# vision-agh/apse_uav

Hardware: AMD Instinct MI355X
Metric: 4K UAV frames/sec (whole node) (higher is better)
Workload: dtype f32

## Files before the change

apse_uav_amd/csrc/apse_common.h:

```cpp
#pragma once
#include <hip/hip_runtime.h>
#include <stdint.h>

#define APSE_OK 0
#define APSE_E_INVALID (-1)
#define APSE_E_HIP (-2)
#define APSE_E_NOMEM (-3)
#define APSE_E_STATE (-4)
#define APSE_E_MISSING (-5)
#define APSE_MAX_FRAME_W 49152
#define APSE_MAX_FRAME_H 32768
#define APSE_MAX_CLASSES 80
#define APSE_LDS_BYTES 163840

typedef __attribute__((ext_vector_type(16))) float f32x16;
typedef __attribute__((ext_vector_type(4))) float f32x4;

struct ConvParams {
    const float* x;
    const float* w;
    const uint16_t* w16;
    const float* bias;
    const float* res;
    float* y;
    float* ws;
    int* tile_cnt;
    const int* m_count;
    int m_per_item;
    int m_hint;
    int B, H, W, cin_log2;
    int OH, OW, Cout;
    int KH, KW, stride, pad;
    int KWCp;
    int M;
    int relu;
    int res_mode;
    int out_mode;
    int y_ld, y_coff;
    int cdec;
    int splitk;
    int steps_total;
    const void* next_w;
    unsigned next_w_bytes;
    int prec;
    int x_st, res_st, y_st;
    int no_stream;
};

int apse_launch_conv(const ConvParams& p, int cfg, hipStream_t s, hipEvent_t ev0 = nullptr, hipEvent_t ev1 = nullptr);
int apse_conv_pick_cfg(int M, int Cout, int steps, int* splitk);
#define APSE_CFG_STREAM 9
#define APSE_CFG_BNECK 10
#define APSE_CFG_GLDS 11
#define APSE_CFG_STEMPOOL 12
#define APSE_CFG_SKINNY 13
#define APSE_NCFG 14
bool apse_conv1x1_stream_ok(const ConvParams& p);
int apse_launch_conv1x1_stream(const ConvParams& p, hipStream_t s, hipEvent_t ev0 = nullptr, hipEvent_t ev1 = nullptr);
bool apse_conv_glds16_ok(const ConvParams& p);
bool apse_conv_glds16_small(const ConvParams& p);
bool apse_conv_skinny_ok(const ConvParams& p);
int apse_launch_conv_skinny(const ConvParams& p, hipStream_t s, hipEvent_t ev0 = nullptr, hipEvent_t ev1 = nullptr);
int apse_launch_conv_glds16(const ConvParams& p, hipStream_t s, hipEvent_t ev0 = nullptr, hipEvent_t ev1 = nullptr);
int apse_conv_effective_cfg(const ConvParams& p, int cfg);
typedef __bf16 bf16x8 __attribute__((ext_vector_type(8)));

#ifdef __HIPCC__
typedef _Float16 f16x4_t __attribute__((ext_vector_type(4)));
typedef __bf16 bf16x4_t __attribute__((ext_vector_type(4)));
__device__ __forceinline__ f32x4 apse_ld4(const void* base, size_t idx, int st) {
    if (st == 0) return *reinterpret_cast<const f32x4*>(reinterpret_cast<const float*>(base) + idx);
    f32x4 r;
    if (st == 1) {
        const uint2 raw = *reinterpret_cast<const uint2*>(reinterpret_cast<const uint16_t*>(base) + idx);
        r[0] = __uint_as_float(raw.x << 16); r[1] = __uint_as_float(raw.x & 0xffff0000u);
        r[2] = __uint_as_float(raw.y << 16); r[3] = __uint_as_float(raw.y & 0xffff0000u);
    } else {
        const f16x4_t h = *reinterpret_cast<const f16x4_t*>(reinterpret_cast<const uint16_t*>(base) + idx);
        r[0] = (float)h[0]; r[1] = (float)h[1]; r[2] = (float)h[2]; r[3] = (float)h[3];
    }
    return r;
}
#ifndef APSE_NT
#define APSE_NT 1
#endif
#if APSE_NT
#define APSE_NT_STORE(v, ptr) __builtin_nontemporal_store(v, ptr)
#else
#define APSE_NT_STORE(v, ptr) (*(ptr) = (v))
#endif
__device__ __forceinline__ float apse_relu(float x) {
    float r;
    asm("v_max_f32 %0, 0, %1" : "=v"(r) : "v"(x));
    return r;
}
__device__ __forceinline__ void apse_st4(void* base, size_t idx, f32x4 v, int st) {
    if (st == 0) { APSE_NT_STORE(v, reinterpret_cast<f32x4*>(reinterpret_cast<float*>(base) + idx)); return; }
    if (st == 1) {
        bf16x4_t b;
        b[0] = (__bf16)v[0]; b[1] = (__bf16)v[1]; b[2] = (__bf16)v[2]; b[3] = (__bf16)v[3];
        APSE_NT_STORE(b, reinterpret_cast<bf16x4_t*>(reinterpret_cast<uint16_t*>(base) + idx));
    } else {
        f16x4_t h;
        h[0] = (_Float16)v[0]; h[1] = (_Float16)v[1]; h[2] = (_Float16)v[2]; h[3] = (_Float16)v[3];
        APSE_NT_STORE(h, reinterpret_cast<f16x4_t*>(reinterpret_cast<uint16_t*>(base) + idx));
    }
}
struct ApseWarm { f32x4 v[4]; };
__device__ __forceinline__ void apse_warm_issue(ApseWarm& wv, const void* w, unsigned bytes, unsigned blk, unsigned nblk, int tid) {
    const unsigned stride = (bytes / nblk + 1023u) & ~1023u;
    const unsigned len = stride > 16384u ? 16384u : stride;
    const unsigned lo = blk * stride;
#pragma unroll
    for (int i = 0; i < 4; ++i) {
        const unsigned o = (unsigned)(i * 256 + tid) * 16u;
        wv.v[i] = f32x4{0.f, 0.f, 0.f, 0.f};
        if (w && o < len && lo + o + 16u <= bytes) wv.v[i] = *reinterpret_cast<const f32x4*>(reinterpret_cast<const char*>(w) + lo + o);
    }
}
__device__ __forceinline__ void apse_warm_retire(ApseWarm& wv) {
#pragma unroll
    for (int i = 0; i < 4; ++i) asm volatile("" ::"v"(wv.v[i]));
}
typedef float f32x8 __attribute__((ext_vector_type(8)));
typedef _Float16 f16x8_t __attribute__((ext_vector_type(8)));

__device__ __forceinline__ f32x8 apse_cvt8(const uint4 raw, int st) {
    f32x8 r;
    if (st == 1) {
        r[0] = __uint_as_float(raw.x << 16); r[1] = __uint_as_float(raw.x & 0xffff0000u);
        r[2] = __uint_as_float(raw.y << 16); r[3] = __uint_as_float(raw.y & 0xffff0000u);
        r[4] = __uint_as_float(raw.z << 16); r[5] = __uint_as_float(raw.z & 0xffff0000u);
        r[6] = __uint_as_float(raw.w << 16); r[7] = __uint_as_float(raw.w & 0xffff0000u);
    } else {
        f16x8_t h;
        __builtin_memcpy(&h, &raw, 16);
#pragma unroll
        for (int k = 0; k < 8; ++k) r[k] = (float)h[k];
    }
    return r;
}

__device__ __forceinline__ void apse_st8(void* base, size_t idx, const f32x8& v, int st) {
    if (st == 0) {
        apse_st4(base, idx, f32x4{v[0], v[1], v[2], v[3]}, 0);
        apse_st4(base, idx + 4, f32x4{v[4], v[5], v[6], v[7]}, 0);
    } else if (st == 1) {
// ... 22 lines not shown
```

apse_uav_amd/csrc/detector.hip:

```cpp
#include "apse_common.h"
#include "../../include/apse_hip.h"
#include "preproc_pixel.h"

#include <math.h>
#include <stdio.h>
#include <string.h>

#include <map>
#include <mutex>
#include <string>
#include <vector>

struct RpnLevel { const float* head; int H, W, stride; int n; int k; float base[3][4]; };
struct RpnLevels { RpnLevel lv[5]; int head_ld; int pre_topk; };
struct TopkJob { int kind; int level; int begin, count; int nsrc; int src[4]; int src_count[4]; int dst; int dst_count; };
struct FpnMaps { const void* p[4]; int H[4], W[4]; float scale[4]; int st; };
struct PasteParams {
    const float* boxes; const int* cls; const int* total; const float* logits; int M, ldc; float sx, sy; int out_h, out_w;
    int words_per_row; float thresh; float* boxes_out; int* valid; int* rect; uint64_t* bits; unsigned long long* sums;
};
extern "C" {
int apse_k_pil_resize(const uint8_t*, uint8_t*, void*, int, uint8_t*, const int*, const int*, int, const int*, const int*, int, int,
                      int, int, int, int, int, int, const float*, const UndistortParams*, const LabTables*, const void*, const int*, int, hipStream_t);
int apse_k_undistort_build_map_compact(const UndistortParams*, void*, int*, hipStream_t);
int apse_k_chw_norm(const float*, void*, int, int, int, int, int, int, const float*, hipStream_t);
int apse_k_maxpool3x3s2(const void*, void*, int, int, int, int, int, hipStream_t);
bool apse_assoc_fc_ok(int K, int N);
int apse_k_assoc_fc(const float*, const float*, const float*, float*, const int*, int, int, int, float*, float*, hipStream_t);
int apse_k_stem_pool16(const void*, const uint16_t*, const float*, void*, int, int, int, int, hipStream_t, hipEvent_t, hipEvent_t);
int apse_k_subsample2(const void*, void*, int, int, int, int, int, hipStream_t);
int apse_k_bottleneck64_fused16(const void*, const void*, void*, const uint16_t*, const float*, const uint16_t*, const float*,
                                const uint16_t*, const float*, int, int, int, int, int, hipStream_t, hipEvent_t, hipEvent_t);
int apse_k_nhwc_to_nchw(const void*, float*, int, int, int, int, hipStream_t);
int apse_k_rpn_topk_stage(const RpnLevels*, const TopkJob*, int, uint64_t*, int, int, uint32_t*, hipStream_t);
int apse_k_rpn_decode(const RpnLevels*, int, const uint64_t*, int, const int*, float, float, float, float*, float*, int*,
                      uint32_t*, int, int, hipStream_t);
int apse_k_nms_percat(const float*, const float*, const int*, int, int, int, const uint32_t*, float, int*, int*, int,
                      void*, int, int, int, hipStream_t);
size_t apse_nms_scratch_bytes(int slots);
int apse_k_rank_final(const float*, const float*, int, const int*, const int*, int, int, float*, float*, int*, int*, uint32_t*,
                      int, hipStream_t);
int apse_k_box_candidates(const float*, int, int, const float*, const int*, int, float, float, float, const float*, float,
                          float*, float*, int*, uint32_t*, float*, int, hipStream_t);
int apse_k_box_candidates_wide(const float*, int, int, const float*, const int*, int, float, float, float, const float*, float,
                               float*, float*, int*, uint32_t*, float*, int*, int*, int, hipStream_t);
int apse_k_nms_lists(const float*, const float*, int, const int*, int*, int, const uint32_t*, float, int*, int*, int, void*, int,
                     hipStream_t);
int apse_k_rank_wide(const float*, const float*, int, const int*, const int*, int, int, float*, float*, int*, int*, int, hipStream_t);
int apse_k_pack_detections(const float*, const float*, const int*, const int*, int, int, int, float*, float*, int*, int*,
                           int*, int*, int*, unsigned long long*, hipStream_t);
int apse_k_roi_align(const FpnMaps*, const float*, const int*, const int*, const int*, int, int, int, void*, int, hipStream_t);
int apse_k_roi_pool(const void*, int, int, int, const float*, const int*, const int*, int, int, float, float*, int, int, hipStream_t);
int apse_k_mask_resize(const uint8_t*, int, int, int, int, int, float*, hipStream_t);
int apse_k_round16(const float*, uint16_t*, size_t, int, hipStream_t);
int apse_k_roi_align_masked(const void*, int, int, int, int, const float*, const float*, int, int, int, float, float*, hipStream_t);
int apse_k_l2_normalize(const float*, float*, int, const int*, int, hipStream_t);
int apse_k_sqdist(const float*, const float*, int, int, int, float*, hipStream_t);
int apse_k_mask_paste(const PasteParams*, int, unsigned long long*, int, hipStream_t);
int apse_k_closest_points(const uint64_t*, const int*, const int*, const unsigned long long*, const int*, const int*, const int*, int,
                          int, int, int, int, int*, int*, unsigned long long*, int, hipStream_t);
int apse_k_closest_single(const uint64_t*, int, int, int, float, float, unsigned long long*, hipStream_t);
int apse_k_undistort_gamma(const UndistortParams*, const uint8_t*, uint8_t*, const LabTables*, int, hipStream_t);
int apse_k_bits_to_dense(const uint64_t*, const int*, int, int, int, uint8_t*, hipStream_t);
int apse_k_copy_mask_windows(const uint64_t*, uint64_t*, int, const long long*, const long long*, const int*, const int*, int, hipStream_t);
int apse_k_dense_to_bits(const uint8_t*, int, int, int, uint64_t*, unsigned long long*, hipStream_t);
}

static std::string g_create_error;
#define NMS_SLOT 1024
#define APSE_NARROW_CLASSES 6
#define APSE_EV_HALF 1024
#define APSE_EXPECTED_DETS 8

struct HostW { std::vector<float> v; std::vector<int64_t> shape; };
struct Tens { float* p = nullptr; int H = 0, W = 0, C = 0; int st = 0; };

struct ConvStep {
    ConvParams p;
    int b_mult = 1;
    int fixed_items = 0;
    int cfg = 0;
    double flops_per_item = 0;
    int count_kind = 0;
    void* pool_y = nullptr;
    std::string name;
};
enum StepKind { S_CONV, S_MAXPOOL, S_SUBSAMPLE, S_BNECK };
struct Step { StepKind kind; ConvStep c; const float* x; float* y; int H, W, C; int st = 0; ConvParams p2, p3; };

struct apse_ctx {
    apse_config cfg;
    std::string err;
    std::map<std::string, HostW> hw;
    bool finalized = false;
    int PH = 0, PW = 0;
    std::vector<void*> allocs;
    std::map<std::string, Tens> t;
    std::vector<Step> backbone, rpnhead, boxhead, maskhead, embedfc;
    float* ws = nullptr; size_t ws_floats = 0; int* tile_cnt = nullptr;
    int *hb = nullptr, *hc = nullptr, *vb = nullptr, *vc = nullptr; int hk = 0, vk = 0; uint8_t* rs_tmp = nullptr;
    int rs_pitch = 0;
    int* hcT = nullptr;
    RpnLevels rl_host; RpnLevels* rl_dev = nullptr;
    std::vector<std::vector<TopkJob>> stages; std::vector<TopkJob*> stage_dev; int nslots = 0; uint64_t* lists = nullptr;
    int final_slot_host[5]; int* final_slot_dev = nullptr;
    float *dec_boxes = nullptr, *dec_scores = nullptr; int* dec_valid = nullptr; uint32_t* maxc = nullptr;
    int *keep_idx = nullptr, *keep_cnt = nullptr; void* nms_scratch = nullptr;
    float *props = nullptr, *prop_scores = nullptr; int *prop_entry = nullptr;
    FpnMaps fm;
    float *cand_boxes = nullptr, *cand_scores = nullptr, *probs = nullptr; int* cand_valid = nullptr;
    int pred_ld = 32;
    bool wide = false;
    int *cls_list = nullptr, *cls_cnt = nullptr;
    float *det_boxes = nullptr, *det_scores = nullptr; int *det_entry = nullptr, *det_cnt = nullptr;
    apse_results_layout lay; uint8_t* res = nullptr;
    uint64_t* bits2[2] = {nullptr, nullptr}; int bits_cur = 0, bits_read = 0;
    unsigned long long* sums = nullptr; int wpr = 0; bool sums_dirty = false;
    float* emb_raw = nullptr;
    float* ws_assoc = nullptr;
    float* rf_mask = nullptr; size_t rf_mask_floats = 0;
    bool box_maxc_clean = false;
    UndistortParams cam; bool cam_on = false; LabTables* cam_lut = nullptr; void* cam_map = nullptr; bool cam_map_ok = false;
    int hint_total = 8;
    hipEvent_t read_ev = nullptr; void* read_pending = nullptr;
    uint8_t* given_host[2] = {nullptr, nullptr}; hipEvent_t given_ev[2] = {nullptr, nullptr}; int given_k = 0;
    bool prof_on = false; std::vector<hipEvent_t> ev_pool; int ev_used = 0;
    struct Pending { int cfg; double flops_per_item; int count_kind; int b_mult; int batch; int e0, e1; };
    std::vector<Pending> pending; double prof[APSE_NCFG][3] = {{0}};
    int ev_base = 0, cal_read = -1; std::vector<Pending> pending_read;
    uint64_t* op_bits = nullptr; unsigned long long* op_sums = nullptr; size_t op_bits_words = 0;
};

static int fail(apse_ctx* c, int code, const std::string& msg) {
    if (c) c->err = msg; else g_create_error = msg;
    return code;
}
#define HIPCHK(c, call)                                                                        \
    do {                                                                                       \
        hipError_t e_ = (call);                                                                \
        if (e_ != hipSuccess) return fail(c, APSE_E_HIP, std::string(#call) + ": " + hipGetErrorString(e_)); \
    } while (0)

template <typename T>
static T* dalloc(apse_ctx* c, size_t n, bool zero = true) {
    void* p = nullptr;
    if (hipMalloc(&p, n * sizeof(T) > 0 ? n * sizeof(T) : 16) != hipSuccess) return nullptr;
    if (zero) hipMemset(p, 0, n * sizeof(T));
    c->allocs.push_back(p);
    return reinterpret_cast<T*>(p);
}
template <typename T>
static T* dupload(apse_ctx* c, const std::vector<T>& v) {
    T* p = dalloc<T>(c, v.size(), false);
    if (p && !v.empty()) hipMemcpy(p, v.data(), v.size() * sizeof(T), hipMemcpyHostToDevice);
    return p;
}

static void pack_oihw(const float* w, int Cout, int Cin, int KH, int KW, int cin_p, const float* scale, float* out,
                      int KWCp) {
    for (int o = 0; o < Cout; ++o) {
        const float sc = scale ? scale[o] : 1.0f;
        for (int r = 0; r < KH; ++r)
            for (int s = 0; s < KW; ++s)
                for (int ci = 0; ci < Cin; ++ci)
                    out[((size_t)o * KH + r) * KWCp + s * cin_p + ci] = w[(((size_t)o * Cin + ci) * KH + r) * KW + s] * sc;
    }
}
static int pow2_at_least(int v) { int p = 4; while (p < v) p <<= 1; return p; }

static const HostW* getw(apse_ctx* c, const std::string& n) {
    auto it = c->hw.find(n);
    return it == c->hw.end() ? nullptr : &it->second;
}

static Tens make_t(apse_ctx* c, const std::string& name, int items, int H, int W, int C, int st = 0) {
    Tens t;
    t.H = H; t.W = W; t.C = C; t.st = st;
    const size_t elems = (size_t)items * H * W * C;
    t.p = dalloc<float>(c, st ? (elems + 1) / 2 : elems);
    c->t[name] = t;
    return t;
}

struct ConvSpec {
    std::string name; std::vector<std::string> wnames;
    int KH, KW, stride, pad, relu;
    int fc_h = 0, fc_w = 0;
    int deconv = 0;
    int s2d = 0;
};

static uint16_t round16(float v, int dtype) {
    if (dtype == 2) {
        const _Float16 hval = (_Float16)v;
        uint16_t r;
        memcpy(&r, &hval, 2);
        return r;
    }
    uint32_t b;
    memcpy(&b, &v, 4);
    if ((b & 0x7fffffffu) > 0x7f800000u) return (uint16_t)((b >> 16) | 0x40);
    return (uint16_t)((b + 0x7fffu + ((b >> 16) & 1u)) >> 16);
}
static int storage_type(const apse_ctx* c) { return (c->cfg.compute_dtype >= 1 && c->cfg.storage16) ? c->cfg.compute_dtype : 0; }

static int add_conv(apse_ctx* c, std::vector<Step>& plan, const ConvSpec& sp, const Tens& in, int in_items_mult, Tens* out,
                    const std::string& out_name, const Tens* res, int res_mode, int y_ld_override, int count_kind,
                    float* out_ptr_override = nullptr, const Tens* out_view = nullptr) {
    std::vector<float> rows;
    std::vector<float> bias;
    int Cout = 0, Cin = 0;
    const int KH = sp.KH, KW = sp.KW;
    for (const auto& wn : sp.wnames) {
        const HostW* w = getw(c, wn + ".weight");
        if (!w) return fail(c, APSE_E_MISSING, "missing weight " + wn + ".weight");
        int co, ci;
        std::vector<float> oihw;
        if (sp.fc_h > 0) {
            co = (int)w->shape[0];
            const int flat = (int)w->shape[1];
            ci = flat / (sp.fc_h * sp.fc_w);
            oihw = w->v;
        } else if (sp.deconv) {
            ci = (int)w->shape[0];
            const int cc = (int)w->shape[1];
            co = 4 * cc;
            oihw.assign((size_t)co * ci, 0.f);
            for (int i = 0; i < ci; ++i)
                for (int o = 0; o < cc; ++o)
                    for (int dy = 0; dy < 2; ++dy)
                        for (int dx = 0; dx < 2; ++dx)
                            oihw[((size_t)((dy * 2 + dx) * cc + o)) * ci + i] = w->v[(((size_t)i * cc + o) * 2 + dy) * 2 + dx];
        } else if (w->shape.size() == 2) {
            co = (int)w->shape[0]; ci = (int)w->shape[1]; oihw = w->v;
        } else if (sp.s2d) {
            if (w->shape.size() != 4 || w->shape[2] != 7 || w->shape[3] != 7 || w->shape[1] != 3 || KH != 4 || KW != 4)
                return fail(c, APSE_E_INVALID, "space-to-depth stem needs a 7x7 filter over 3 channels: " + wn);
            co = (int)w->shape[0]; ci = 12;
            oihw.assign((size_t)co * 12 * 16, 0.f);
            for (int o = 0; o < co; ++o)
                for (int ch = 0; ch < 3; ++ch)
                    for (int r = 0; r < 4; ++r)
                        for (int sx = 0; sx < 4; ++sx)
                            for (int dy = 0; dy < 2; ++dy)
                                for (int dx = 0; dx < 2; ++dx) {
                                    const int ky = 2 * r + dy - 1, kx = 2 * sx + dx - 1;
                                    if (ky < 0 || ky > 6 || kx < 0 || kx > 6) continue;
                                    oihw[(((size_t)o * 12 + (dy * 2 + dx) * 3 + ch) * 4 + r) * 4 + sx] = w->v[(((size_t)o * 3 + ch) * 7 + ky) * 7 + kx];
                                }
        } else {
            co = (int)w->shape[0]; ci = (int)w->shape[1]; oihw = w->v;
            if ((int)w->shape[2] != KH || (int)w->shape[3] != KW) return fail(c, APSE_E_INVALID, "kernel size mismatch " + wn);
        }
        if (Cin && ci != Cin) return fail(c, APSE_E_INVALID, "Cin mismatch in fused conv " + sp.name);
        Cin = ci;
        const HostW* g = getw(c, wn + ".norm.weight");
        std::vector<float> scale;
        const int nb = sp.deconv ? co / 4 : co;
        std::vector<float> b(nb, 0.f);
        if (g) {
            const HostW* be = getw(c, wn + ".norm.bias");
            const HostW* mu = getw(c, wn + ".norm.running_mean");
            const HostW* var = getw(c, wn + ".norm.running_var");
            if (!be || !mu || !var) return fail(c, APSE_E_MISSING, "incomplete norm for " + wn);
            scale.resize(co);
            for (int o = 0; o < co; ++o) {
                scale[o] = g->v[o] * (1.0f / sqrtf(var->v[o] + 1e-5f));
                b[o] = be->v[o] - mu->v[o] * scale[o];
            }
            const size_t per = (size_t)ci * KH * KW;
            for (int o = 0; o < co; ++o)
                for (size_t k = 0; k < per; ++k) oihw[(size_t)o * per + k] *= scale[o];
        } else {
            const HostW* bw = getw(c, wn + ".bias");
            if (bw) for (int o = 0; o < nb; ++o) b[o] = bw->v[o];
        }
        rows.insert(rows.end(), oihw.begin(), oihw.end());
        bias.insert(bias.end(), b.begin(), b.end());
        Cout += co;
    }
    const int cin_p = in.C;
    if (pow2_at_least(Cin) != cin_p && Cin != cin_p) return fail(c, APSE_E_INVALID, "input channels mismatch at " + sp.name);
    if (sp.s2d && (in.C != 16 || sp.stride != 1 || sp.pad != 2)) return fail(c, APSE_E_INVALID, "space-to-depth stem geometry");
    const int KWC = KW * cin_p, KWCp = apse_roundup(KWC, 32);
    const int Cout_p = apse_roundup(Cout, 128);
    std::vector<float> packed((size_t)Cout_p * KH * KWCp, 0.f);
    pack_oihw(rows.data(), Cout, Cin, KH, KW, cin_p, nullptr, packed.data(), KWCp);
    std::vector<float> bias_p(Cout_p, 0.f);
    for (size_t i = 0; i < bias.size(); ++i) bias_p[i] = bias[i];
    const bool use_bf16 = (c->cfg.compute_dtype >= 1 && Cout > 32 && sp.name != "assoc_fc" && sp.name != "box_pred" &&
                           sp.name != "mask_logits");
    float* wd = nullptr;
    uint16_t* wd16 = nullptr;
    if (use_bf16) {
        std::vector<uint16_t> p16(packed.size());
        for (size_t i = 0; i < packed.size(); ++i) p16[i] = round16(packed[i], c->cfg.compute_dtype);
        wd16 = dupload(c, p16);
    } else {
        wd = dupload(c, packed);
    }
    float* bd = dupload(c, bias_p);
    if ((!wd && !wd16) || !bd) return fail(c, APSE_E_NOMEM, "weight upload failed at " + sp.name);

    Step st;
    st.kind = S_CONV;
    ConvStep& cs = st.c;
    memset(&cs.p, 0, sizeof(cs.p));
    cs.name = sp.name;
    cs.b_mult = in_items_mult;
    cs.count_kind = count_kind;
    ConvParams& p = cs.p;
    p.x = in.p; p.w = wd; p.w16 = wd16; p.bias = bd; p.res = res ? res->p : nullptr; p.res_mode = res_mode;
    p.x_st = in.st; p.res_st = res ? res->st : 0;
    p.H = in.H; p.W = in.W; p.cin_log2 = apse_ilog2(cin_p);
    p.KH = KH; p.KW = KW; p.stride = sp.stride; p.pad = sp.pad; p.KWCp = KWCp;
    p.OH = (in.H + 2 * sp.pad - KH) / sp.stride + 1;
    p.OW = (in.W + 2 * sp.pad - KW) / sp.stride + 1;
    if (sp.s2d) { p.OH = in.H; p.OW = in.W; }
    p.Cout = Cout; p.relu = sp.relu;
    p.steps_total = KH * (KWCp / 32);
    p.splitk = 1;
    p.out_mode = sp.deconv ? 1 : 0;
    p.prec = use_bf16 ? c->cfg.compute_dtype : 0;
    p.cdec = sp.deconv ? Cout / 4 : 0;
    const int out_c = sp.deconv ? Cout / 4 : (y_ld_override > 0 ? y_ld_override : Cout);
    const int oh = sp.deconv ? 2 * p.OH : p.OH, ow = sp.deconv ? 2 * p.OW : p.OW;
    const int out_st = out_view ? out_view->st : ((use_bf16 && !out_ptr_override) ? storage_type(c) : 0);
    if (out_st && (out_c & 7)) return fail(c, APSE_E_INVALID, "16-bit tensors need C % 8 == 0 at " + sp.name);
    Tens o;
    if (out_view) { o = *out_view; o.H = oh; o.W = ow; o.C = out_c; c->t[out_name] = o; }
    else if (out_ptr_override) { o.p = out_ptr_override; o.H = oh; o.W = ow; o.C = out_c; }
    else o = make_t(c, out_name, c->cfg.max_batch * in_items_mult, oh, ow, out_c, out_st);
    p.y_st = o.st;
    if (!o.p) return fail(c, APSE_E_NOMEM, "activation alloc failed at " + sp.name);
    p.y = o.p; p.y_ld = out_c; p.y_coff = 0;
    cs.flops_per_item = sp.s2d ? 2.0 * p.OH * p.OW * (double)Cout * 7 * 7 * 3
                               : 2.0 * p.OH * p.OW * (double)Cout * KH * KW * Cin;
    const int Mfull = c->cfg.max_batch * in_items_mult * p.OH * p.OW;
    int sk = 1;
    cs.cfg = apse_conv_pick_cfg(Mfull, Cout, p.steps_total, &sk);
    if (count_kind == 2) {
        const int kd = c->cfg.dets_per_image < APSE_EXPECTED_DETS ? c->cfg.dets_per_image : APSE_EXPECTED_DETS;
        const int rows = kd * c->cfg.max_batch * p.OH * p.OW;
        sk = 1;
        cs.cfg = apse_conv_pick_cfg(rows < Mfull ? rows : Mfull, Cout, p.steps_total, &sk);
    }
    p.splitk = sk;
    if (sk > 1) {
        const size_t need = (size_t)sk * Mfull * Cout;
        if (need > c->ws_floats) c->ws_floats = need;
    }
    if (out) *out = o;
    plan.push_back(st);
    return APSE_OK;
}

static int run_plan(apse_ctx* c, std::vector<Step>& plan, int batch, hipStream_t s) {
    int* total_dev = reinterpret_cast<int*>(c->res + c->lay.total);
    int* propcnt_dev = reinterpret_cast<int*>(c->res + c->lay.prop_count);
    for (size_t si = 0; si < plan.size(); ++si) {
        Step& st = plan[si];
        int rc = APSE_OK;
        if (st.kind == S_CONV) {
            ConvParams p = st.c.p;
            for (size_t sj = si + 1; sj < plan.size() && sj <= si + 2; ++sj)
                if (plan[sj].kind == S_CONV) {
                    const ConvParams& q = plan[sj].c.p;
                    const size_t elems = (size_t)apse_roundup(q.Cout, 128) * q.KH * q.KWCp;
                    p.next_w = q.w16 ? (const void*)q.w16 : (const void*)q.w;
                    const size_t bytes = elems * (q.w16 ? 2 : 4);
                    p.next_w_bytes = bytes > (64u << 20) ? (64u << 20) : (unsigned)bytes;
                    break;
                }
            p.B = st.c.fixed_items > 0 ? st.c.fixed_items : batch * st.c.b_mult;
            p.M = p.B * p.OH * p.OW;
            p.ws = c->ws;
            p.tile_cnt = nullptr;
            p.m_count = nullptr; p.m_per_item = p.OH * p.OW; p.m_hint = 0;
            int cfg = st.c.cfg;
            if (st.c.count_kind == 2) {
                p.m_count = total_dev;
                const int mh = (c->hint_total > 0 ? c->hint_total : 1) * p.m_per_item;
                p.m_hint = mh < p.M ? mh : p.M;
                if (p.prec != 0 && p.splitk == 1 && (cfg == 0 || cfg == 1 || cfg == 3)) {
                    int sk_dyn = 1;
                    const int cfg_dyn = apse_conv_pick_cfg(p.m_hint, p.Cout, p.steps_total, &sk_dyn);
                    if (sk_dyn == 1 && (cfg_dyn == 0 || cfg_dyn == 1 || cfg_dyn == 3)) cfg = cfg_dyn;
                }
            }
            else if (st.c.count_kind == 1 && batch == 1) p.m_count = propcnt_dev;
            int e0 = -1;
            if (c->prof_on && c->ev_used == 0) {
                hipEventRecord(c->ev_pool[c->ev_base], s);
                hipEventRecord(c->ev_pool[c->ev_base + 1], s);
                c->ev_used = 2;
            }
            if (c->prof_on && c->ev_used + 2 <= APSE_EV_HALF) { e0 = c->ev_base + c->ev_used; c->ev_used += 2; }
            if (st.c.pool_y) {
                rc = apse_k_stem_pool16(p.x, p.w16, p.bias, st.c.pool_y, batch, p.H, p.W, p.prec, s, e0 >= 0 ? c->ev_pool[e0] : nullptr,
                                        e0 >= 0 ? c->ev_pool[e0 + 1] : nullptr);
                cfg = APSE_CFG_STEMPOOL;
            } else {
                rc = apse_launch_conv(p, cfg, s, e0 >= 0 ? c->ev_pool[e0] : nullptr, e0 >= 0 ? c->ev_pool[e0 + 1] : nullptr);
                cfg = apse_conv_effective_cfg(p, cfg);
            }
            if (e0 >= 0) c->pending.push_back({cfg, st.c.flops_per_item, st.c.count_kind, st.c.b_mult, batch, e0, e0 + 1});
        } else if (st.kind == S_BNECK) {
            int e0 = -1;
            if (c->prof_on && c->ev_used == 0) {
                hipEventRecord(c->ev_pool[c->ev_base], s);
                hipEventRecord(c->ev_pool[c->ev_base + 1], s);
                c->ev_used = 2;
            }
            if (c->prof_on && c->ev_used + 2 <= APSE_EV_HALF) { e0 = c->ev_base + c->ev_used; c->ev_used += 2; }
            const ConvParams& q1 = st.c.p;
            rc = apse_k_bottleneck64_fused16(st.x, st.p3.res, st.y, q1.w16, q1.bias, st.p2.w16, st.p2.bias, st.p3.w16, st.p3.bias, batch,
                                             st.H, st.W, st.C, st.st, s, e0 >= 0 ? c->ev_pool[e0] : nullptr, e0 >= 0 ? c->ev_pool[e0 + 1] : nullptr);
            if (e0 >= 0) c->pending.push_back({APSE_CFG_BNECK, st.c.flops_per_item, 0, 1, batch, e0, e0 + 1});
        } else if (st.kind == S_MAXPOOL) {
            rc = apse_k_maxpool3x3s2(st.x, st.y, batch, st.H, st.W, st.C, st.st, s);
        } else {
            rc = apse_k_subsample2(st.x, st.y, batch, st.H, st.W, st.C, st.st, s);
        }
        if (rc != APSE_OK) return fail(c, rc, "launch failed at step " + st.c.name);
    }
    return APSE_OK;
}

static void layout_results(apse_ctx* c) {
    apse_results_layout& L = c->lay;
    memset(&L, 0, sizeof(L));
    const int B = c->cfg.max_batch, kd = c->cfg.dets_per_image, n = B * kd, E = c->cfg.embed_dim;
    L.n_max = n; L.dets_per_image = kd; L.embed_dim = E; L.max_batch = B;
    size_t o = 0;
    auto take = [&](size_t bytes) { size_t r = o; o += (bytes + 15) / 16 * 16; return r; };
    L.total = take(4);
    L.offset = take(4 * (B + 1));
    L.prop_count = take(4 * B);
    L.img = take(4 * n); L.cls = take(4 * n); L.roi = take(4 * n); L.score = take(4 * n);
    L.box_resized = take(16 * n); L.box = take(16 * n); L.valid = take(4 * n); L.rect = take(16 * n);
    L.mass = take(4 * n); L.centroid = take(8 * n);
    L.closest = take((size_t)8 * n * kd);
    L.embedding = take((size_t)4 * n * E);
    L.bytes = o;
}

static int build_plan(apse_ctx* c) {
    const apse_config& g = c->cfg;
    const int B = g.max_batch;
    c->PH = apse_roundup(g.image_h, 32);
    c->PW = apse_roundup(g.image_w, 32);
    layout_results(c);
    c->res = dalloc<uint8_t>(c, c->lay.bytes);
    if (!c->res) return fail(c, APSE_E_NOMEM, "results alloc");
    int rc;
    Tens cur;
    bool fused_stem = false;
    if (storage_type(c)) {
        Tens x0 = make_t(c, "input", B, c->PH / 2, c->PW / 2, 16, storage_type(c));
        ConvSpec sp{"stem.conv1", {"backbone.bottom_up.stem.conv1"}, 4, 4, 1, 2, 1};
        sp.s2d = 1;
        if (!getenv("APSE_NO_STEM_FUSE")) {
            Tens pooled = make_t(c, "stem", B, (x0.H + 2 - 3) / 2 + 1, (x0.W + 2 - 3) / 2 + 1, 64, storage_type(c));
            if (!pooled.p) return fail(c, APSE_E_NOMEM, "stem alloc");
            Tens unused;
            rc = add_conv(c, c->backbone, sp, x0, 1, &unused, "stem.conv1", nullptr, 0, 0, 0, nullptr, &pooled);
            if (rc) return rc;
            c->t.erase("stem.conv1");
            c->backbone.back().c.pool_y = pooled.p;
            cur = pooled;
            fused_stem = true;
        } else {
            rc = add_conv(c, c->backbone, sp, x0, 1, &cur, "stem.conv1", nullptr, 0, 0, 0);
        }
    } else {
        Tens x0 = make_t(c, "input", B, c->PH, c->PW, 4);
        rc = add_conv(c, c->backbone, ConvSpec{"stem.conv1", {"backbone.bottom_up.stem.conv1"}, 7, 7, 2, 3, 1}, x0, 1, &cur,
                      "stem.conv1", nullptr, 0, 0, 0);
    }
    if (rc) return rc;
    if (!fused_stem) {
        Step st; st.kind = S_MAXPOOL; st.x = cur.p; st.H = cur.H; st.W = cur.W; st.C = cur.C;
        Tens o = make_t(c, "stem", B, (cur.H + 2 - 3) / 2 + 1, (cur.W + 2 - 3) / 2 + 1, cur.C, cur.st);
        st.y = o.p; st.c.name = "stem.pool"; st.st = cur.st;
// ... 217 lines not shown
    for (int i = 1; i <= 4; ++i) {
        char nm[48], wn[64];
        snprintf(nm, sizeof nm, "mask_fcn%d", i);
        snprintf(wn, sizeof wn, "roi_heads.mask_head.mask_fcn%d", i);
        Tens o;
        rc = add_conv(c, c->maskhead, ConvSpec{nm, {wn}, 3, 3, 1, 1, 1}, m, KD, &o, nm, nullptr, 0, 0, 2);
        if (rc) return rc;
        m = o;
    }
    {
        ConvSpec sp{"mask_deconv", {"roi_heads.mask_head.deconv"}, 1, 1, 1, 0, 1};
        sp.deconv = 1;
        rc = add_conv(c, c->maskhead, sp, m, KD, &md, "mask_deconv", nullptr, 0, 0, 2);
        if (rc) return rc;
    }
    rc = add_conv(c, c->maskhead, ConvSpec{"mask_logits", {"roi_heads.mask_head.predictor"}, 1, 1, 1, 0, 0}, md, KD, &ml,
                  "mask_logits", nullptr, 0, 0, 2);
    if (rc) return rc;
    c->wpr = (g.frame_w + 63) / 64;
    for (int k = 0; k < 2; ++k) c->bits2[k] = dalloc<uint64_t>(c, (size_t)NM * g.frame_h * c->wpr, false);
    c->sums = dalloc<unsigned long long>(c, (size_t)NM * 3);
    if (!c->bits2[0] || !c->bits2[1]) return fail(c, APSE_E_NOMEM, "mask bit planes alloc");
    const int R = g.assoc_roi;
    Tens ap = make_t(c, "assoc_pooled", NM, R, R, 256);
    Tens er;
    {
        ConvSpec sp{"assoc_fc", {"association.fc"}, R, R, 1, 0, 0, R, R};
        c->emb_raw = dalloc<float>(c, (size_t)NM * g.embed_dim);
        rc = add_conv(c, c->embedfc, sp, ap, KD, &er, "assoc_fc", nullptr, 0, 0, 2, c->emb_raw);
        if (rc) return rc;
        const ConvParams& fp = c->embedfc[0].c.p;
        if (fp.w && fp.KWCp == R * 256 && apse_assoc_fc_ok(fp.KH * fp.KWCp, g.embed_dim) && !getenv("APSE_NO_ASSOC_FC")) {
            c->ws_assoc = dalloc<float>(c, (size_t)(fp.KH * fp.KWCp / 128) * NM * g.embed_dim, false);
            if (!c->ws_assoc) return fail(c, APSE_E_NOMEM, "association FC workspace");
        }
    }
    if (c->ws_floats) {
        c->ws = dalloc<float>(c, c->ws_floats, false);
        if (!c->ws) return fail(c, APSE_E_NOMEM, "split-K workspace alloc");
    }
    c->tile_cnt = dalloc<int>(c, 65536);
    c->rs_pitch = (g.image_w * 3 + 15) & ~15;
    c->rs_tmp = dalloc<uint8_t>(c, (size_t)B * g.frame_h * c->rs_pitch, false);
    hipError_t e = hipDeviceSynchronize();
    if (e != hipSuccess) return fail(c, APSE_E_HIP, std::string("plan build: ") + hipGetErrorString(e));
    return APSE_OK;
}

extern "C" {

#ifndef APSE_SRC_HASH
#define APSE_SRC_HASH "unknown"
#endif
const char* apse_version(void) { return "apse_hip 0.6 (gfx950, f32 / bf16 / f16 MFMA) src " APSE_SRC_HASH; }

int apse_create(const apse_config* cfg, apse_ctx** out) {
    if (!cfg || !out) return fail(nullptr, APSE_E_INVALID, "null argument");
    if (cfg->struct_size != (int)sizeof(apse_config)) return fail(nullptr, APSE_E_INVALID, "apse_config size mismatch");
    if (cfg->max_batch < 1 || cfg->max_batch > 64 || cfg->rpn_pre_topk > 1000 || cfg->rpn_post_topk > 1000 ||
        cfg->dets_per_image > 100 || cfg->num_classes < 1 || cfg->num_classes > APSE_MAX_CLASSES || cfg->embed_dim > 256 ||
        cfg->max_batch * cfg->dets_per_image > 1024)
        return fail(nullptr, APSE_E_INVALID, "config out of supported range");
    {
        const double t = cfg->score_thresh;
        const double per_roi = t > 0.0 ? ceil(1.0 / t) - 1.0 : (double)cfg->num_classes;
        const double bound = (double)cfg->rpn_post_topk * (per_roi < cfg->num_classes ? per_roi : (double)cfg->num_classes);
        if (bound >= 40000.0)
            return fail(nullptr, APSE_E_INVALID,
                        "box candidate bound rpn_post_topk * min(num_classes, ceil(1 / score_thresh) - 1) = " +
                            std::to_string((long long)bound) + " reaches 40000, where detectron2's batched_nms changes method");
    }
    if (cfg->frame_h < 1 || cfg->frame_w < 1 || cfg->frame_h > APSE_MAX_FRAME_H || cfg->frame_w > APSE_MAX_FRAME_W)
        return fail(nullptr, APSE_E_INVALID, "frame size out of supported range (1 <= frame_h <= " + std::to_string(APSE_MAX_FRAME_H) +
                                             ", 1 <= frame_w <= " + std::to_string(APSE_MAX_FRAME_W) + ")");
    if (cfg->compute_dtype < 0 || cfg->compute_dtype > 2 || (cfg->compute_dtype && !cfg->storage16))
        return fail(nullptr, APSE_E_INVALID, "compute_dtype 1 / 2 (bf16 / f16 matrix cores) needs storage16 = 1: the f32-storage variant "
                                             "of the 16-bit modes was removed in round 4 (no BASELINE configuration uses it)");
    int ndev = 0;
    if (hipGetDeviceCount(&ndev) != hipSuccess || ndev <= 0)
        return fail(nullptr, APSE_E_HIP, "no HIP device visible: the apse_uav hot path has no CPU fallback");
    if (hipSetDevice(cfg->device) != hipSuccess) return fail(nullptr, APSE_E_HIP, "hipSetDevice failed");
    apse_ctx* c = new apse_ctx();
    c->cfg = *cfg;
    *out = c;
    return APSE_OK;
}

void apse_destroy(apse_ctx* c) {
    if (!c) return;
    hipSetDevice(c->cfg.device);
    for (void* p : c->allocs) hipFree(p);
    if (c->rf_mask) hipFree(c->rf_mask);
    if (c->read_ev) hipEventDestroy(c->read_ev);
    for (int k = 0; k < 2; ++k) {
        if (c->given_ev[k]) hipEventDestroy(c->given_ev[k]);
        if (c->given_host[k]) hipHostFree(c->given_host[k]);
    }
    delete c;
}

const char* apse_last_error(apse_ctx* c) { return c ? c->err.c_str() : g_create_error.c_str(); }

int apse_set_weight(apse_ctx* c, const char* name, const float* host, const int64_t* shape, int ndim) {
    if (!c || !name || !host || !shape || ndim < 1 || ndim > 4) return fail(c, APSE_E_INVALID, "bad weight argument");
    if (c->finalized) return fail(c, APSE_E_STATE, "weights already finalized");
    HostW w;
    size_t n = 1;
    for (int i = 0; i < ndim; ++i) { w.shape.push_back(shape[i]); n *= (size_t)shape[i]; }
    w.v.assign(host, host + n);
    c->hw[name] = std::move(w);
    return APSE_OK;
}

int apse_finalize_weights(apse_ctx* c) {
    if (!c) return APSE_E_INVALID;
    if (c->finalized) return fail(c, APSE_E_STATE, "already finalized");
    hipSetDevice(c->cfg.device);
    int rc = build_plan(c);
    if (rc) return rc;
    c->hw.clear();
    c->finalized = true;
    return APSE_OK;
}

int apse_set_resize_tables(apse_ctx* c, const int* hb, const int* hc, int hk, const int* vb, const int* vc, int vk) {
    if (!c || !hb || !hc || !vb || !vc) return fail(c, APSE_E_INVALID, "null table");
    const apse_config& g = c->cfg;
    std::vector<int> a(hb, hb + 2 * g.image_w), b(hc, hc + (size_t)hk * g.image_w), d(vb, vb + 2 * g.image_h),
        e(vc, vc + (size_t)vk * g.image_h);
    for (int i = 0; i < g.image_w; ++i)
        if (a[2 * i] < 0 || a[2 * i + 1] > hk || a[2 * i] + a[2 * i + 1] > g.frame_w) return fail(c, APSE_E_INVALID, "bad horizontal bounds");
    for (int i = 0; i < g.image_h; ++i)
        if (d[2 * i] < 0 || d[2 * i + 1] > vk || d[2 * i] + d[2 * i + 1] > g.frame_h) return fail(c, APSE_E_INVALID, "bad vertical bounds");
    c->hb = dupload(c, a); c->hc = dupload(c, b); c->vb = dupload(c, d); c->vc = dupload(c, e);
    c->hk = hk; c->vk = vk;
    c->hcT = nullptr;
    if (hk <= 8) {
        std::vector<int> t((size_t)8 * g.image_w, 0);
        for (int i = 0; i < g.image_w; ++i)
            for (int j = 0; j < a[2 * i + 1] && j < hk; ++j) t[(size_t)j * g.image_w + i] = b[(size_t)i * hk + j];
        c->hcT = dupload(c, t);
    }
    return APSE_OK;
}

#define NEED_READY(c, batch)                                                                     \
    if (!(c) || !(c)->finalized) return fail(c, APSE_E_STATE, "weights not finalized");          \
    if ((batch) < 1 || (batch) > (c)->cfg.max_batch) return fail(c, APSE_E_INVALID, "batch out of range");

int apse_preprocess_frames(apse_ctx* c, const uint8_t* frames, int batch, void* stream) {
    NEED_READY(c, batch);
    if (!c->hb) return fail(c, APSE_E_STATE, "resize tables not set");
    const apse_config& g = c->cfg;
    int rc = apse_k_pil_resize(frames, c->rs_tmp, c->t["input"].p, c->t["input"].st, nullptr, c->hb, c->hc, c->hk, c->vb, c->vc, c->vk, batch,
                               g.frame_h, g.frame_w, g.image_h, g.image_w, c->PH, c->PW, g.pixel_mean, c->cam_on ? &c->cam : nullptr, c->cam_lut, c->cam_map_ok ? c->cam_map : nullptr,
                               c->hcT, c->rs_pitch, (hipStream_t)stream);
    return rc ? fail(c, rc, "pil resize launch failed") : APSE_OK;
}

int apse_preprocess_images(apse_ctx* c, const float* images, int batch, void* stream) {
    NEED_READY(c, batch);
    const apse_config& g = c->cfg;
    int rc = apse_k_chw_norm(images, c->t["input"].p, c->t["input"].st, batch, g.image_h, g.image_w, c->PH, c->PW, g.pixel_mean,
                             (hipStream_t)stream);
    return rc ? fail(c, rc, "chw normalise launch failed") : APSE_OK;
}
// ... 711 lines not shown
```

Before: 173.0.

## Add Winograd F(2x2,3x3) MFMA kernel for selected f32 3x3 convolutions

Adds a Winograd F(2,3) f32 convolution kernel that transforms input tiles in registers, runs 16 batched GEMMs on f32 MFMA with double-buffered LDS, and applies the output transform, bias and ReLU in the epilogue. Filters are pre-transformed on the host at plan time and used for the FPN output 2/3 and RPN t2/t3 layers when enough blocks exist. It is meant to cut the multiply count of 3x3 stride-1 convolutions by about 2.25x. In exchange it adds a new code path with slightly different rounding and larger transformed weight buffers, and it can be disabled through an environment variable.

After: 185.8 (median of 6 runs). +7.4%, better.

```diff
diff --git a/apse_uav_amd/csrc/apse_common.h b/apse_uav_amd/csrc/apse_common.h
--- a/apse_uav_amd/csrc/apse_common.h
+++ b/apse_uav_amd/csrc/apse_common.h
@@ -45,6 +45,7 @@
     int prec;
     int x_st, res_st, y_st;
     int no_stream;
+    const float* wu;
 };
 
 int apse_launch_conv(const ConvParams& p, int cfg, hipStream_t s, hipEvent_t ev0 = nullptr, hipEvent_t ev1 = nullptr);
@@ -63,6 +64,9 @@
 int apse_launch_conv_skinny(const ConvParams& p, hipStream_t s, hipEvent_t ev0 = nullptr, hipEvent_t ev1 = nullptr);
 int apse_launch_conv_glds16(const ConvParams& p, hipStream_t s, hipEvent_t ev0 = nullptr, hipEvent_t ev1 = nullptr);
 int apse_conv_effective_cfg(const ConvParams& p, int cfg);
+bool apse_conv_winograd_ok(const ConvParams& p, int max_items);
+int apse_conv_winograd_blocks(const ConvParams& p);
+int apse_launch_conv_winograd(const ConvParams& p, hipStream_t s, hipEvent_t ev0 = nullptr, hipEvent_t ev1 = nullptr);
 typedef __bf16 bf16x8 __attribute__((ext_vector_type(8)));
 
 #ifdef __HIPCC__
diff --git a/apse_uav_amd/csrc/conv_winograd.hip b/apse_uav_amd/csrc/conv_winograd.hip
--- /dev/null
+++ b/apse_uav_amd/csrc/conv_winograd.hip
@@ -0,0 +1,201 @@
+#include "apse_common.h"
+
+namespace {
+constexpr int WTR = 16, WTC = 4;
+constexpr int WT = WTR * WTC;
+constexpr int WN = 64;
+constexpr int KC = 8;
+constexpr int NTHR = 512;
+constexpr int SLICE_F = 16 * WT * KC;
+constexpr size_t WINO_LDS = (size_t)2 * 2 * SLICE_F * sizeof(float);
+static_assert(WN == WT, "V and U slices share one size");
+static_assert((size_t)16 * WT * 32 * sizeof(float) <= WINO_LDS, "epilogue chunk must fit the staging LDS");
+}
+
+__global__ __launch_bounds__(NTHR) void conv_winograd_f32(const ConvParams p) {
+    extern __shared__ __attribute__((aligned(16))) char smem[];
+    float* Vs = reinterpret_cast<float*>(smem);
+    float* Us = Vs + 2 * SLICE_F;
+    float* Cs = reinterpret_cast<float*>(smem);
+
+    const int tid = threadIdx.x;
+    const int lane = tid & 63, wave = tid >> 6;
+    const int fr = lane & 31, fh = lane >> 5;
+
+    const int tiles_y = (p.OH + 2 * WTR - 1) / (2 * WTR), tiles_x = (p.OW + 2 * WTC - 1) / (2 * WTC);
+    const int nblk = p.Cout / WN;
+    const int nwg = p.B * tiles_y * tiles_x * nblk;
+    int bid;
+    {
+        const int wg = blockIdx.x;
+        const int q = nwg >> 3, r = nwg & 7, xcd = wg & 7, idx = wg >> 3;
+        bid = (xcd < r ? xcd * (q + 1) : r * (q + 1) + (xcd - r) * q) + idx;
+    }
+    const int nb = bid % nblk;
+    int rest = bid / nblk;
+    const int bx = rest % tiles_x; rest /= tiles_x;
+    const int by = rest % tiles_y;
+    const int b = rest / tiles_y;
+    const int oy0 = by * 2 * WTR, ox0 = bx * 2 * WTC, n0 = nb * WN;
+    const int C = 1 << p.cin_log2;
+    const int nsteps = C / KC;
+
+    const int cg = tid & 1, t = (tid >> 1) & (WT - 1), ti = tid >> 7;
+    const int ra = ti == 0 ? 0 : (ti == 2 ? 2 : 1);
+    const int rb = ti == 0 ? 2 : (ti == 1 ? 2 : (ti == 2 ? 1 : 3));
+    const int iy_a = oy0 + 2 * (t / WTC) - 1 + ra, iy_b = oy0 + 2 * (t / WTC) - 1 + rb;
+    const int ix0 = ox0 + 2 * (t % WTC) - 1;
+    const __amdgpu_buffer_rsrc_t xrsrc =
+        __builtin_amdgcn_make_buffer_rsrc(const_cast<float*>(p.x), 0, (int)((((unsigned)(p.B * p.H * p.W)) << p.cin_log2) * 4u), 0x00020000);
+    unsigned xoff[2][4];
+#pragma unroll
+    for (int r = 0; r < 2; ++r) {
+        const int iy = r ? iy_b : iy_a;
+#pragma unroll
+        for (int c = 0; c < 4; ++c) {
+            const int ix = ix0 + c;
+            const bool in = (unsigned)iy < (unsigned)p.H && (unsigned)ix < (unsigned)p.W;
+            xoff[r][c] = in ? ((((unsigned)((b * p.H + iy) * p.W + ix)) << p.cin_log2) + (unsigned)(cg * 4)) * 4u : 0x80000000u;
+        }
+    }
+    const float* ubase = p.wu + (size_t)n0 * KC;
+    const size_t ustep = (size_t)16 * p.Cout * KC;
+
+    f32x4 xr[2][4], ur[4];
+    auto fetch = [&](int s) {
+        const unsigned kb = (unsigned)(s * KC * 4);
+#pragma unroll
+        for (int r = 0; r < 2; ++r)
+#pragma unroll
+            for (int c = 0; c < 4; ++c)
+                xr[r][c] = __builtin_bit_cast(f32x4, __builtin_amdgcn_raw_buffer_load_b128(xrsrc, (int)(xoff[r][c] + kb), 0, 0));
+        const float* us = ubase + (size_t)s * ustep;
+#pragma unroll
+        for (int k = 0; k < 4; ++k) {
+            const int q = tid + NTHR * k;
+            const int xi = q >> 7, co = (q >> 1) & 63, h = q & 1;
+            ur[k] = *reinterpret_cast<const f32x4*>(us + ((size_t)xi * p.Cout + co) * KC + h * 4);
+        }
+    };
+    auto stage = [&](int buf) {
+        f32x4 x[4];
+#pragma unroll
+        for (int c = 0; c < 4; ++c) x[c] = ti == 1 ? xr[0][c] + xr[1][c] : xr[0][c] - xr[1][c];
+        const f32x4 v[4] = {x[0] - x[2], x[1] + x[2], x[2] - x[1], x[1] - x[3]};
+        const int sw = (cg ^ ((t >> 3) & 1)) * 4;
+#pragma unroll
+        for (int j = 0; j < 4; ++j)
+            *reinterpret_cast<f32x4*>(Vs + buf * SLICE_F + ((4 * ti + j) * WT + t) * KC + sw) = v[j];
+#pragma unroll
+        for (int k = 0; k < 4; ++k) {
+            const int q = tid + NTHR * k;
+            const int xi = q >> 7, co = (q >> 1) & 63, h = q & 1;
+            *reinterpret_cast<f32x4*>(Us + buf * SLICE_F + (xi * WN + co) * KC + ((h ^ ((co >> 3) & 1)) * 4)) = ur[k];
+        }
+    };
+
+    f32x16 acc[2][2][2];
+#pragma unroll
+    for (int a = 0; a < 2; ++a)
+#pragma unroll
+        for (int i = 0; i < 2; ++i)
+#pragma unroll
+            for (int j = 0; j < 2; ++j)
+#pragma unroll
+                for (int v = 0; v < 16; ++v) acc[a][i][j][v] = 0.f;
+
+    fetch(0);
+    stage(0);
+    __syncthreads();
+    const int fsw = (fh ^ ((fr >> 3) & 1)) * 4;
+    for (int s = 0; s < nsteps; ++s) {
+        const int buf = s & 1;
+        const bool more = s + 1 < nsteps;
+        if (more) fetch(s + 1);
+#pragma unroll
+        for (int a = 0; a < 2; ++a) {
+            const int xi = 2 * wave + a;
+            f32x4 af[2], bf[2];
+#pragma unroll
+            for (int i = 0; i < 2; ++i) af[i] = *reinterpret_cast<const f32x4*>(Vs + buf * SLICE_F + (xi * WT + 32 * i + fr) * KC + fsw);
+#pragma unroll
+            for (int j = 0; j < 2; ++j) bf[j] = *reinterpret_cast<const f32x4*>(Us + buf * SLICE_F + (xi * WN + 32 * j + fr) * KC + fsw);
+#pragma unroll
+            for (int k = 0; k < 4; ++k)
+#pragma unroll
+                for (int i = 0; i < 2; ++i)
+#pragma unroll
+                    for (int j = 0; j < 2; ++j)
+                        acc[a][i][j] = __builtin_amdgcn_mfma_f32_32x32x2f32(af[i][k], bf[j][k], acc[a][i][j], 0, 0, 0);
+        }
+        if (more) stage(buf ^ 1);
+        __syncthreads();
+    }
+
+    const int et = tid >> 3, eg = tid & 7;
+    const int oy = oy0 + 2 * (et / WTC), ox = ox0 + 2 * (et % WTC);
+    typedef unsigned u32x4_t __attribute__((ext_vector_type(4)));
+#pragma unroll
+    for (int j = 0; j < 2; ++j) {
+#pragma unroll
+        for (int a = 0; a < 2; ++a)
+#pragma unroll
+            for (int i = 0; i < 2; ++i)
+#pragma unroll
+                for (int v = 0; v < 16; ++v) {
+                    const int row = 32 * i + (v & 3) + 8 * (v >> 2) + 4 * fh;
+                    Cs[((2 * wave + a) * WT + row) * 32 + fr] = acc[a][i][j][v];
+                }
+        __syncthreads();
+        f32x4 m[16];
+#pragma unroll
+        for (int k = 0; k < 16; ++k) m[k] = *reinterpret_cast<const f32x4*>(Cs + (k * WT + et) * 32 + eg * 4);
+        f32x4 s0[4], s1[4];
+#pragma unroll
+        for (int c = 0; c < 4; ++c) {
+            s0[c] = m[c] + m[4 + c] + m[8 + c];
+            s1[c] = m[4 + c] - m[8 + c] - m[12 + c];
+        }
+        const int co = n0 + 32 * j + 4 * eg;
+        const f32x4 bias4 = p.bias ? *reinterpret_cast<const f32x4*>(p.bias + co) : f32x4{0.f, 0.f, 0.f, 0.f};
+        f32x4 y[2][2] = {{s0[0] + s0[1] + s0[2], s0[1] - s0[2] - s0[3]}, {s1[0] + s1[1] + s1[2], s1[1] - s1[2] - s1[3]}};
+#pragma unroll
+        for (int dy = 0; dy < 2; ++dy)
+#pragma unroll
+            for (int dx = 0; dx < 2; ++dx) {
+                f32x4 val = y[dy][dx] + bias4;
+                if (p.relu) {
+#pragma unroll
+                    for (int k = 0; k < 4; ++k) val[k] = apse_relu(val[k]);
+                }
+                if (oy + dy < p.OH && ox + dx < p.OW)
+                    APSE_NT_STORE(val, reinterpret_cast<f32x4*>(p.y + ((size_t)(b * p.OH + oy + dy) * p.OW + ox + dx) * p.y_ld + p.y_coff + co));
+            }
+        __syncthreads();
+    }
+}
+
+bool apse_conv_winograd_ok(const ConvParams& p, int max_items) {
+    return p.prec == 0 && p.x_st == 0 && p.y_st == 0 && p.KH == 3 && p.KW == 3 && p.stride == 1 && p.pad == 1 && p.out_mode == 0 &&
+           p.res_mode == 0 && p.splitk == 1 && p.Cout % WN == 0 && p.cin_log2 >= 3 && p.OH == p.H && p.OW == p.W &&
+           (p.y_ld & 3) == 0 && (p.y_coff & 3) == 0 && ((((size_t)max_items * p.H * p.W) << p.cin_log2) * 4 < 0x7fff0000ull);
+}
+
+int apse_conv_winograd_blocks(const ConvParams& p) {
+    return ((p.OH + 2 * WTR - 1) / (2 * WTR)) * ((p.OW + 2 * WTC - 1) / (2 * WTC)) * (p.Cout / WN);
+}
+
+int apse_launch_conv_winograd(const ConvParams& p, hipStream_t s, hipEvent_t ev0, hipEvent_t ev1) {
+    if (!p.wu || !apse_conv_winograd_ok(p, p.B) || p.m_count) return APSE_E_INVALID;
+    static bool attr_done = false;
+    if (!attr_done) {
+        hipFuncSetAttribute(reinterpret_cast<const void*>(&conv_winograd_f32), hipFuncAttributeMaxDynamicSharedMemorySize, (int)WINO_LDS);
+        attr_done = true;
+    }
+    const int tiles_y = (p.OH + 2 * WTR - 1) / (2 * WTR), tiles_x = (p.OW + 2 * WTC - 1) / (2 * WTC);
+    const int grid = p.B * tiles_y * tiles_x * (p.Cout / WN);
+    if (ev0) hipEventRecord(ev0, s);
+    hipLaunchKernelGGL(conv_winograd_f32, dim3(grid), dim3(NTHR), WINO_LDS, s, p);
+    if (ev1) hipEventRecord(ev1, s);
+    return hipGetLastError() == hipSuccess ? APSE_OK : APSE_E_HIP;
+}
diff --git a/apse_uav_amd/csrc/detector.hip b/apse_uav_amd/csrc/detector.hip
--- a/apse_uav_amd/csrc/detector.hip
+++ b/apse_uav_amd/csrc/detector.hip
@@ -70,6 +70,7 @@
 #define NMS_SLOT 1024
 #define APSE_NARROW_CLASSES 6
 #define APSE_EV_HALF 1024
+#define APSE_WINO_MIN_BLOCKS 128
 #define APSE_EXPECTED_DETS 8
 
 struct HostW { std::vector<float> v; std::vector<int64_t> shape; };
@@ -91,6 +92,7 @@
 struct apse_ctx {
     apse_config cfg;
     std::string err;
+    bool f32_winograd = true;
     std::map<std::string, HostW> hw;
     bool finalized = false;
     int PH = 0, PW = 0;
@@ -203,6 +205,27 @@
     return (uint16_t)((b + 0x7fffu + ((b >> 16) & 1u)) >> 16);
 }
 static int storage_type(const apse_ctx* c) { return (c->cfg.compute_dtype >= 1 && c->cfg.storage16) ? c->cfg.compute_dtype : 0; }
+
+static bool winograd_layer(const std::string& n) {
+    return n == "backbone.fpn_output2" || n == "backbone.fpn_output3" || n == "rpn_t2" || n == "rpn_t3";
+}
+static std::vector<float> winograd_filters(const float* oihw, int Cout, int Cin, int cin_p) {
+    static const double G[4][3] = {{1, 0, 0}, {0.5, 0.5, 0.5}, {0.5, -0.5, 0.5}, {0, 0, 1}};
+    std::vector<float> u((size_t)16 * Cout * cin_p, 0.f);
+    for (int o = 0; o < Cout; ++o)
+        for (int ci = 0; ci < Cin; ++ci) {
+            const float* g = oihw + ((size_t)o * Cin + ci) * 9;
+            double t[4][3];
+            for (int i = 0; i < 4; ++i)
+                for (int s = 0; s < 3; ++s) t[i][s] = G[i][0] * g[s] + G[i][1] * g[3 + s] + G[i][2] * g[6 + s];
+            for (int i = 0; i < 4; ++i)
+                for (int j = 0; j < 4; ++j) {
+                    const double v = t[i][0] * G[j][0] + t[i][1] * G[j][1] + t[i][2] * G[j][2];
+                    u[(((size_t)(ci / 8) * 16 + 4 * i + j) * Cout + o) * 8 + (ci & 7)] = (float)v;
+                }
+        }
+    return u;
+}
 
 static int add_conv(apse_ctx* c, std::vector<Step>& plan, const ConvSpec& sp, const Tens& in, int in_items_mult, Tens* out,
                     const std::string& out_name, const Tens* res, int res_mode, int y_ld_override, int count_kind,
@@ -350,6 +373,11 @@
         const size_t need = (size_t)sk * Mfull * Cout;
         if (need > c->ws_floats) c->ws_floats = need;
     }
+    if (c->f32_winograd && winograd_layer(sp.name) && count_kind == 0 && apse_conv_winograd_ok(p, c->cfg.max_batch * in_items_mult) &&
+        apse_conv_winograd_blocks(p) >= APSE_WINO_MIN_BLOCKS) {
+        p.wu = dupload(c, winograd_filters(rows.data(), Cout, Cin, cin_p));
+        if (!p.wu) return fail(c, APSE_E_NOMEM, "weight upload failed at " + sp.name);
+    }
     if (out) *out = o;
     plan.push_back(st);
     return APSE_OK;
@@ -366,8 +394,8 @@
             for (size_t sj = si + 1; sj < plan.size() && sj <= si + 2; ++sj)
                 if (plan[sj].kind == S_CONV) {
                     const ConvParams& q = plan[sj].c.p;
-                    const size_t elems = (size_t)apse_roundup(q.Cout, 128) * q.KH * q.KWCp;
-                    p.next_w = q.w16 ? (const void*)q.w16 : (const void*)q.w;
+                    const size_t elems = q.wu ? (size_t)16 * q.Cout * (1 << q.cin_log2) : (size_t)apse_roundup(q.Cout, 128) * q.KH * q.KWCp;
+                    p.next_w = q.w16 ? (const void*)q.w16 : (q.wu ? (const void*)q.wu : (const void*)q.w);
                     const size_t bytes = elems * (q.w16 ? 2 : 4);
                     p.next_w_bytes = bytes > (64u << 20) ? (64u << 20) : (unsigned)bytes;
                     break;
@@ -400,6 +428,8 @@
                 rc = apse_k_stem_pool16(p.x, p.w16, p.bias, st.c.pool_y, batch, p.H, p.W, p.prec, s, e0 >= 0 ? c->ev_pool[e0] : nullptr,
                                         e0 >= 0 ? c->ev_pool[e0 + 1] : nullptr);
                 cfg = APSE_CFG_STEMPOOL;
+            } else if (p.wu) {
+                rc = apse_launch_conv_winograd(p, s, e0 >= 0 ? c->ev_pool[e0] : nullptr, e0 >= 0 ? c->ev_pool[e0 + 1] : nullptr);
             } else {
                 rc = apse_launch_conv(p, cfg, s, e0 >= 0 ? c->ev_pool[e0] : nullptr, e0 >= 0 ? c->ev_pool[e0 + 1] : nullptr);
                 cfg = apse_conv_effective_cfg(p, cfg);
@@ -783,6 +813,10 @@
     if (hipSetDevice(cfg->device) != hipSuccess) return fail(nullptr, APSE_E_HIP, "hipSetDevice failed");
     apse_ctx* c = new apse_ctx();
     c->cfg = *cfg;
+    {
+        const char* e = getenv("APSE_F32_WINOGRAD");
+        c->f32_winograd = !(e && atoi(e) == 0);
+    }
     *out = c;
     return APSE_OK;
 }
diff --git a/apse_uav_amd/winograd.py b/apse_uav_amd/winograd.py
--- /dev/null
+++ b/apse_uav_amd/winograd.py
@@ -0,0 +1,53 @@
+import numpy as np
+
+BT = np.array([[1, 0, -1, 0], [0, 1, 1, 0], [0, -1, 1, 0], [0, 1, 0, -1]], dtype=np.float64)
+G = np.array([[1, 0, 0], [0.5, 0.5, 0.5], [0.5, -0.5, 0.5], [0, 0, 1]], dtype=np.float64)
+AT = np.array([[1, 1, 1, 0], [0, 1, -1, -1]], dtype=np.float64)
+
+
+def filter_transform(w):
+    w = np.asarray(w, dtype=np.float64)
+    u = np.einsum("ir,ocrs,js->ijoc", G, w, G)
+    return u.reshape(16, w.shape[0], w.shape[1]).astype(np.float32)
+
+
+def _input_transform(d):
+    d0, d1, d2, d3 = d[..., 0, :, :], d[..., 1, :, :], d[..., 2, :, :], d[..., 3, :, :]
+    rows = [d0 - d2, d1 + d2, d2 - d1, d1 - d3]
+    v = []
+    for x in rows:
+        x0, x1, x2, x3 = x[..., 0, :], x[..., 1, :], x[..., 2, :], x[..., 3, :]
+        v += [x0 - x2, x1 + x2, x2 - x1, x1 - x3]
+    return np.stack(v, axis=-2)
+
+
+def _output_transform(m):
+    q = [m[..., k, :] for k in range(16)]
+    s0 = [q[0 + j] + q[4 + j] + q[8 + j] for j in range(4)]
+    s1 = [q[4 + j] - q[8 + j] - q[12 + j] for j in range(4)]
+    y00 = s0[0] + s0[1] + s0[2]
+    y01 = s0[1] - s0[2] - s0[3]
+    y10 = s1[0] + s1[1] + s1[2]
+    y11 = s1[1] - s1[2] - s1[3]
+    return np.stack([np.stack([y00, y01], -2), np.stack([y10, y11], -2)], -3)
+
+
+def emulate(x_hwc, w_oihw, bias, relu):
+    x = np.asarray(x_hwc, dtype=np.float32)
+    H, W, C = x.shape
+    th, tw = (H + 1) // 2, (W + 1) // 2
+    xp = np.zeros((2 * th + 2, 2 * tw + 2, C), np.float32)
+    xp[1:H + 1, 1:W + 1] = x
+    iy = (2 * np.arange(th))[:, None] + np.arange(4)[None, :]
+    ix = (2 * np.arange(tw))[:, None] + np.arange(4)[None, :]
+    d = xp[iy[:, None, :, None], ix[None, :, None, :]]
+    v = _input_transform(d)
+    u = filter_transform(w_oihw)
+    m = np.zeros((th, tw, 16, u.shape[1]), np.float32)
+    for c in range(C):
+        m += v[..., c:c + 1] * u[None, None, :, :, c]
+    y = _output_transform(m) + np.asarray(bias, np.float32)
+    if relu:
+        y = np.maximum(y, 0)
+    y = y.transpose(0, 2, 1, 3, 4).reshape(2 * th, 2 * tw, -1)
+    return y[:H, :W]
```
